# piotrprzybyszdev/Path-Tracing

Measured on AMD Instinct MI355X. Metric: Msamples/s (paths*spp/s) at 1920x1080, 8spp, depth 8, higher is better.
Workload: dtype f32; 1 GPU; chess_like (procedural stand-in for BASELINE configs[1] 'Khronos ABeautifulGame'), 1920x1080, 8 spp, depth 8; triangles=1999000, frames_in_flight=8, parallelism=pixel-tile shard x1, backend=wavefront, tile=32

## Files before the change

### path-tracing_amd/csrc/pt_bvh.hpp

```cpp
#pragma once

#include "pt_device.hpp"

namespace ptd
{

constexpr int kNodeWidth = 4;
struct BvhNode
{
    float4 a;
    int4 refs;
    uint4 q0;
    uint4 q1;
};
static_assert(sizeof(BvhNode) == 64, "BvhNode is 64 B");
constexpr int kEmptyRef = 0x7ffffffe;
constexpr int kRefDone = 0x7fffffff;
constexpr int kRefNone = 0x7ffffffd;

struct Tri
{
    float4 a;
    float4 b;
    float4 c;
};
static_assert(sizeof(Tri) == 48, "Tri is 48 B");
constexpr uint32_t kTriNonOpaque = 0x80000000u;
constexpr uint32_t kLeafNonOpaque = 0x40000000u, kLeafSlotMask = 0x3fffffffu;
constexpr uint32_t kMaxTriangles = 0x3fffffffu;

struct Hit
{
    float t, u, v;
    uint32_t pair, prim;
    uint32_t slot;
};


constexpr uint32_t kRefillMin = 16;
constexpr int kLdsStack = 16;
constexpr int kLdsStackMega = 64;
constexpr int kGlobalSpill = 80;
constexpr uint32_t kMaxPersistentThreads = 2048u * 256u;
constexpr uint32_t kMaxNodeVisits = 1u << 20;

struct AlphaTri
{
    float4 a;
    float4 b;
};
struct AlphaTex
{
// ... 288 lines not shown
#endif
            if (kMaskWalk)
            {
                PT_ENTER_UNORDERED(h, r0, r1, r2, r3, st, ref, kRefNone, push)
            }
            else
            {
                if (h > 3) st.push((uint32_t)r3);
                if (h > 2) st.push((uint32_t)r2);
                if (h > 1) st.push((uint32_t)r1);
                ref = h > 0 ? r0 : kRefNone;
            }
            if (STATS && stackDepth && (uint32_t)st.sp > *stackDepth)
                *stackDepth = (uint32_t)st.sp;
            if (ref == kRefNone)
            {
                if (st.sp == 0)
                    break;
                ref = (int)st.pop();
            }
        }
        else
        {
            if (STATS)
                (*triTests)++;
            const uint32_t leafSlot = ALPHA ? (uint32_t)~ref & kLeafSlotMask : (uint32_t)~ref;
            const Tri *tp = &sc.tris[leafSlot];
            const float4 ta = tp->a, tb = tp->b, tc = tp->c;
            float t, u, v;
            if (intersectTri(F3(ta.x, ta.y, ta.z), F3(ta.w, tb.x, tb.y), F3(tb.z, tb.w, tc.x), o, d, tmin, tmax, t, u, v) &&
                (!ALPHA || !(__float_as_uint(tc.w) & kTriNonOpaque) ||
                 anyHitKeeps<ANY_HIT>(sc, __float_as_uint(tc.y), __float_as_uint(tc.z), leafSlot, __float_as_uint(tc.w), t, u, v, decal)))
            {
                const uint32_t pair = __float_as_uint(tc.y), prim = __float_as_uint(tc.z);
                if (ANY_HIT)
                {
                    best.pair = pair;
                    best.prim = prim;
                    best.slot = leafSlot;
                    return true;
                }
                if (t < best.t || (t == best.t && (pair < best.pair || (pair == best.pair && prim < best.prim))))
                {
                    best.t = t;
                    best.u = u;
                    best.v = v;
                    best.pair = pair;
                    best.prim = prim;
                    best.slot = leafSlot;
                }
            }
            if (st.sp == 0)
                break;
            ref = (int)st.pop();
        }
    }
    if (ALPHA && decalOut)
        *decalOut = decal;
    return best.pair != 0xffffffffu;
}

constexpr uint32_t kTraceChunk = 128;
constexpr int kNodeStepsPerRound = 2;


#define PT_TMIN (IO::kFixedTmin >= 0.0f ? IO::kFixedTmin : tmin)
#define PT_TMAX (IO::kFixedTmax >= 0.0f ? IO::kFixedTmax : tmax)
template <bool ANY_HIT, bool ALPHA, typename IO>
PT_DEV void persistentTrace(const TraceScene &sc, IO &io, uint32_t count, uint32_t *__restrict__ chunkCounter, Stack &st)
{
    const uint32_t lane = threadIdx.x & 63u;
    const uint64_t below = (1ull << lane) - 1ull;
// ... 108 lines not shown
                }
                else
                {
                    if (kUnordered)
                    {
                        PT_ENTER_UNORDERED(h, r0, r1, r2, r3, st, ref, kRefNone, push)
                    }
                    else
                    {
                        if (h > 3) st.push((uint32_t)r3);
                        if (h > 2) st.push((uint32_t)r2);
                        if (h > 1) st.push((uint32_t)r1);
                        ref = h > 0 ? r0 : kRefNone;
                    }
                    if (ref == kRefNone)
                        ref = st.sp ? (int)st.pop() : kRefDone;
                }
            }
        }

        if (have && ref < 0)
        {
            const uint32_t leafBits = (uint32_t)~ref;
            const uint32_t leafSlot = ALPHA ? leafBits & kLeafSlotMask : leafBits;
            const Tri *tp = &sc.tris[leafSlot];
            const float4 ta = tp->a, tb = tp->b, tc = tp->c;
            float4 aa = make_float4(0.0f, 0.0f, 0.0f, 0.0f), ab = aa;
            const bool nonOpaque = ALPHA && (leafBits & kLeafNonOpaque) != 0u;
            if (nonOpaque)
            {
                aa = sc.alphaTris[leafSlot].a;
                ab = sc.alphaTris[leafSlot].b;
            }
            float t, u, v;
            if (__builtin_expect(st.allInLds(), 1))
                ref = st.sp ? (int)st.popLds() : kRefDone;
            else
                ref = st.sp ? (int)st.pop() : kRefDone;
            bool candidate = intersectTri(F3(ta.x, ta.y, ta.z), F3(ta.w, tb.x, tb.y), F3(tb.z, tb.w, tc.x), o, d, PT_TMIN, PT_TMAX, t, u, v);
            uint32_t pair = __float_as_uint(tc.y), prim = __float_as_uint(tc.z);
            if (ALPHA && candidate && nonOpaque)
            {
                const float alpha = hitAlpha(sc, aa, ab, __float_as_uint(tc.w), u, v);
                candidate = ANY_HIT ? !(alpha < 1.0f) : !(alpha < 0.5f);
                if (!ANY_HIT && !candidate && t <= best.t)
                    io.ignored(t, u, v, leafSlot, sc);
                if (candidate && (!ANY_HIT || IO::kNeedsPrim))
                {
                    const float4 again = sc.tris[fetchAgainAfter(leafSlot, alpha)].c;
                    pair = __float_as_uint(again.y);
                    prim = __float_as_uint(again.z);
                }
            }
            if (candidate)
            {
                if (ANY_HIT)
                {
                    best.pair = IO::kNeedsPrim ? pair : 0u;
                    best.slot = leafSlot;
                    ref = kRefDone;
                }
                else if (t < best.t || (t == best.t && (pair < best.pair || (pair == best.pair && prim < __float_as_uint(sc.tris[io.bestSlot(item)].c.z)))))
                {
// ... 22 lines not shown
```

### path-tracing_amd/csrc/pt_bvh_build.hpp

```cpp
#pragma once

#include "pt_bvh.hpp"

namespace ptd
{


PT_DEV uint32_t orderedFloat(float f)
{
    const uint32_t u = __float_as_uint(f);
    return (u & 0x80000000u) ? ~u : (u | 0x80000000u);
}
PT_DEV float unorderedFloat(uint32_t u)
{
    return __uint_as_float((u & 0x80000000u) ? (u & 0x7fffffffu) : ~u);
}

__global__ void k_tri_setup(uint32_t n, uint32_t pairCount, const uint32_t *__restrict__ pairFirst,
                            const DevPair *__restrict__ pairs, const PtxVertex *__restrict__ vertices,
                            const uint32_t *__restrict__ indices, Tri *__restrict__ triTmp, float4 *__restrict__ boxLo,
                            float4 *__restrict__ boxHi, uint32_t *__restrict__ sceneBounds, uint8_t *__restrict__ inert, int refit)
{
    const uint32_t g = blockIdx.x * blockDim.x + threadIdx.x;
    if (g >= n)
// ... 47 lines not shown
    boxHi[g] = make_float4(h[0], h[1], h[2], 0.0f);
    if (refit)
        return;
    for (int a = 0; a < 3; a++)
    {
        const float c = 0.5f * (l[a] + h[a]);
        const bool ok = !isInert && c == c && fabsf(c) < 3.0e38f;
        uint32_t mn = ok ? orderedFloat(c) : 0xffffffffu, mx = ok ? orderedFloat(c) : 0u;
        const bool fullWave = __ballot(1) == ~0ull;
        if (fullWave)
            for (int o = 32; o > 0; o >>= 1)
            {
                mn = min(mn, (uint32_t)__shfl_xor((int)mn, o));
                mx = max(mx, (uint32_t)__shfl_xor((int)mx, o));
            }
        if (!fullWave || (threadIdx.x & 63u) == 0u)
        {
            if (mn != 0xffffffffu)
                atomicMin(&sceneBounds[a], mn);
            if (mx != 0u)
                atomicMax(&sceneBounds[3 + a], mx);
        }
    }
}

constexpr uint32_t kMaxSplitsPerTri = 64;
constexpr double kSplitPriorityScale = 1048576.0;

struct SplitGrid
{
    float mn[3], cell[3];
};
PT_DEV SplitGrid splitGrid(const uint32_t *sceneBounds, int cubic)
{
    SplitGrid g;
    float widest = 0.0f;
    for (int a = 0; a < 3; a++)
        widest = fmaxf(widest, unorderedFloat(sceneBounds[3 + a]) - unorderedFloat(sceneBounds[a]));
    for (int a = 0; a < 3; a++)
    {
        g.mn[a] = unorderedFloat(sceneBounds[a]);
        const float ext = cubic ? widest : unorderedFloat(sceneBounds[3 + a]) - g.mn[a];
        g.cell[a] = ext > 0.0f ? ext / 2097152.0f : 0.0f;
    }
    return g;
}
// ... 1139 lines not shown
        d[8] = v->Tangent[0]; d[9] = v->Tangent[1]; d[10] = v->Tangent[2];
        d[11] = v->Bitangent[0]; d[12] = v->Bitangent[1]; d[13] = v->Bitangent[2];
        o[k] = loadVertex(v);
    }
    f[42] = f[43] = 0.0f;
    f3 wp[3], wn[3], gn;
    worldCorners(pr, o[0], o[1], o[2], wp, wn, gn);
    for (int k = 0; k < 3; k++)
    {
        f[44 + 3 * k] = wp[k].x; f[45 + 3 * k] = wp[k].y; f[46 + 3 * k] = wp[k].z;
        f[53 + 3 * k] = wn[k].x; f[54 + 3 * k] = wn[k].y; f[55 + 3 * k] = wn[k].z;
    }
    f[62] = gn.x; f[63] = gn.y; f[64] = gn.z;
    f[65] = f[66] = f[67] = 0.0f;
    for (int k = 0; k < 17; k++)
        out->v[k] = make_float4(f[4 * k], f[4 * k + 1], f[4 * k + 2], f[4 * k + 3]);
}

__global__ void k_emit(int n, const uint32_t *__restrict__ vals, const float4 *__restrict__ boxLo,
                       const float4 *__restrict__ boxHi, const int2 *__restrict__ children, const float4 *__restrict__ nodeLo,
                       const float4 *__restrict__ nodeHi, const Tri *__restrict__ triTmp, BvhNode *__restrict__ nodes,
                       Tri *__restrict__ tris, const DevPair *__restrict__ pairs, const PtxVertex *__restrict__ vertices,
                       const uint32_t *__restrict__ indices, ShadeTri *__restrict__ shadeTris, const uint8_t *__restrict__ decide,
                       const uint32_t *__restrict__ refTri)
{
    const int i = blockIdx.x * blockDim.x + threadIdx.x;
    if (i < n)
    {
        const Tri t = triTmp[refTri ? refTri[vals[i]] : vals[i]];
        tris[i] = t;
        writeShadeTri(t, pairs, vertices, indices, &shadeTris[i]);
    }
    if (i >= n - 1)
        return;
    ChildBox c[kNodeWidth];
    int count = 2;
    if (decide)
    {
        int ref[kNodeWidth] = { 0, 0, 0, 0 }, slots[kNodeWidth] = { 0, 0, 0, 0 }, sp = 0, out[kNodeWidth] = { 0, 0, 0, 0 };
        count = 0;
        {
            const int2 ch = children[i];
            const int k = 1 + (int)((decide[i] >> 1) & 3u);
            ref[0] = ch.y; slots[0] = 4 - k;
            ref[1] = ch.x; slots[1] = k;
            sp = 2;
        }
        while (sp > 0)
        {
            sp--;
            const int x = ref[sp], j = slots[sp];
            const uint32_t d = x >= 0 ? decide[x] : 0u;
            if (x < 0 || j == 1 || ((d >> (1 + j)) & 1u))
                out[count++] = x;
// ... 103 lines not shown
                    while (qh < 255 && decodeQ(o[a], qh, scale) < (double)c[k].hi[a])
                        qh++;
                    if (decodeQ(o[a], qh, scale) < (double)c[k].hi[a])
                        ok = false;
                }
                {
                    wl |= ql << (8 * k);
                    wh |= qh << (8 * k);
                }
            }
            if (ok || e >= 254)
            {
                ebits[a] = (uint32_t)e;
                qlo[a] = wl;
                qhi[a] = wh;
                break;
            }
            e++;
        }
    }
    BvhNode nd;
    nd.a = make_float4(o[0], o[1], o[2], __uint_as_float(ebits[0] | (ebits[1] << 8) | (ebits[2] << 16) | (orderAxis << 24)));
    for (int k = 0; k < count; k++)
        if (c[k].ref < 0 && (__float_as_uint(triTmp[refTri ? refTri[vals[~c[k].ref]] : vals[~c[k].ref]].c.w) & kTriNonOpaque))
            c[k].ref = ~(int)((uint32_t)~c[k].ref | kLeafNonOpaque);
    nd.refs = make_int4(c[0].ref, c[1].ref, count > 2 ? c[2].ref : kEmptyRef, count > 3 ? c[3].ref : kEmptyRef);
    nd.q0 = make_uint4(qlo[0], qhi[0], qlo[1], qhi[1]);
    nd.q1 = make_uint4(qlo[2], qhi[2], 0u, 0u);
    nodes[i] = nd;
}

__global__ void __launch_bounds__(256) k_relayout_level(uint32_t lo, uint32_t hi, const BvhNode *__restrict__ raw, uint32_t *__restrict__ oldOf,
                                                        uint32_t *__restrict__ nextFree, BvhNode *__restrict__ out)
{
    const uint32_t i = lo + blockIdx.x * blockDim.x + threadIdx.x, lane = threadIdx.x & 63u;
    BvhNode nd;
    nd.refs = make_int4(kEmptyRef, kEmptyRef, kEmptyRef, kEmptyRef);
    if (i < hi)
        nd = raw[oldOf[i]];
    int refs[kNodeWidth] = { nd.refs.x, nd.refs.y, nd.refs.z, nd.refs.w };
    uint32_t c = 0;
    for (int k = 0; k < kNodeWidth; k++)
        c += (refs[k] >= 0 && refs[k] != kEmptyRef) ? 1u : 0u;
    uint32_t incl = c;
    for (uint32_t d = 1; d < 64; d <<= 1)
    {
        const uint32_t up = __shfl_up(incl, d);
        if (lane >= d)
// ... 41 lines not shown
        pos[0] = 0u;
    for (int k = 0; k < kNodeWidth; k++)
        if (refs[k] >= 0 && refs[k] != kEmptyRef)
        {
            pos[refs[k]] = next;
            next += size[refs[k]];
        }
}
__global__ void k_place_nodes(uint32_t count, const BvhNode *__restrict__ nodes, const uint32_t *__restrict__ pos, BvhNode *__restrict__ out)
{
    const uint32_t i = blockIdx.x * blockDim.x + threadIdx.x;
    if (i >= count)
        return;
    BvhNode nd = nodes[i];
    int refs[kNodeWidth] = { nd.refs.x, nd.refs.y, nd.refs.z, nd.refs.w };
    for (int k = 0; k < kNodeWidth; k++)
        if (refs[k] >= 0 && refs[k] != kEmptyRef)
            refs[k] = (int)pos[refs[k]];
    nd.refs = make_int4(refs[0], refs[1], refs[2], refs[3]);
    out[pos[i]] = nd;
}

__global__ void k_single_leaf_root(const uint32_t *vals, const float4 *boxLo, const float4 *boxHi, const Tri *triTmp, BvhNode *nodes, Tri *tris,
                                   const DevPair *pairs, const PtxVertex *vertices, const uint32_t *indices, ShadeTri *shadeTris)
{
    const uint32_t g = vals[0];
    writeShadeTri(triTmp[g], pairs, vertices, indices, &shadeTris[0]);
    tris[0] = triTmp[g];
    BvhNode nd;
    const float lo[3] = { boxLo[g].x, boxLo[g].y, boxLo[g].z }, hi[3] = { boxHi[g].x, boxHi[g].y, boxHi[g].z };
    uint32_t eb[3];
    for (int a = 0; a < 3; a++)
    {
        int e = 1;
        while (e < 254 && decodeQ(lo[a], 255u, __uint_as_float((uint32_t)e << 23)) < (double)hi[a])
            e++;
        eb[a] = (uint32_t)e;
    }
    nd.a = make_float4(lo[0], lo[1], lo[2], __uint_as_float(eb[0] | (eb[1] << 8) | (eb[2] << 16)));
    nd.refs = make_int4((__float_as_uint(triTmp[g].c.w) & kTriNonOpaque) ? ~(int)kLeafNonOpaque : ~0, kEmptyRef, kEmptyRef, kEmptyRef);
    nd.q0 = make_uint4(0xffffff00u, 0x000000ffu, 0xffffff00u, 0x000000ffu);
    nd.q1 = make_uint4(0xffffff00u, 0x000000ffu, 0u, 0u);
    nodes[0] = nd;
}

__global__ void k_alpha_tris(uint32_t n, Tri *__restrict__ tris, const ShadeTri *__restrict__ shadeTris, SceneView sv,
                             const uint32_t *__restrict__ alphaTexOf, const AlphaTex *__restrict__ alphaTex, AlphaTri *__restrict__ out)
{
    const uint32_t i = blockIdx.x * blockDim.x + threadIdx.x;
    if (i >= n)
        return;
    AlphaTri r;
    r.a = make_float4(0.0f, 0.0f, 0.0f, 0.0f);
    r.b = make_float4(0.0f, 0.0f, 1.0f, __uint_as_float(kNoAlphaTex));
    const float4 tc = tris[i].c;
    if (__float_as_uint(tc.w) & kTriNonOpaque)
    {
        const ShadeTri *st = &shadeTris[i];
        const float4 q0 = st->v[0], q1 = st->v[1], q4 = st->v[4], q7 = st->v[7], q8 = st->v[8];
        r.a = make_float4(q0.w, q1.x, q4.y, q4.z);
        const DevPair *pr = &sv.pairs[__float_as_uint(tc.y)];
        const uint32_t materialType = pr->materialId & 0xffu, materialIndex = pr->materialId >> 8;
        uint32_t idx = 0;
// ... 42 lines not shown
```

### path-tracing_amd/csrc/pt_runtime.hpp

```cpp
#pragma once

#include <algorithm>
#include <atomic>
#include <cstdarg>
#include <cstdio>
#include <cstdlib>
#include <cstring>
#include <string>
#include <vector>

#include "pt_aux_kernels.hpp"
#include "pt_bvh_build.hpp"
#include "pt_post.hpp"


template <typename T> struct DevBuf
{
    T *p = nullptr;
    size_t n = 0;
    DevBuf() = default;
    DevBuf(const DevBuf &) = delete;
    DevBuf &operator=(const DevBuf &) = delete;
    ~DevBuf() { release(); }
    hipError_t alloc(size_t count)
// ... 35 lines not shown
};

struct EnvSwitches
{
    uint32_t cuPartition = 0;
    bool singleStream = false;
    bool verbose = false;
    bool karrasBuilder = false;
    bool plocFixed = false;
    uint32_t plocRadius = 0;
    float plocShape = 0.0f;
    int reinsertPasses = -1;
    float splitBudget = -1.0f;
    int layout = -1;
    int collapse = -1;
    int shadeSort = -1;
    long tailThreshold = -1;
    uint32_t framesPerWave = 8;
    uint32_t raysPerThread = 0;
    long residentCap = -1;
    uint32_t copyGroups = 0;
    bool snapshotMemcpy = false;
    bool fenceRefit = false;
    static EnvSwitches read()
    {
        EnvSwitches e;
        e.verbose = getenv("PTX_VERBOSE") != nullptr;
        if (const char *v = getenv("PTX_COPY_GROUPS"))
            e.copyGroups = (uint32_t)strtoul(v, nullptr, 10);
        e.snapshotMemcpy = getenv("PTX_SNAPSHOT_MEMCPY") != nullptr && std::strcmp(getenv("PTX_SNAPSHOT_MEMCPY"), "0") != 0;
        e.fenceRefit = getenv("PTX_FENCE_REFIT") != nullptr && std::strcmp(getenv("PTX_FENCE_REFIT"), "0") != 0;
        if (const char *v = getenv("PTX_BUILDER"))
            e.karrasBuilder = std::strcmp(v, "lbvh") == 0;
        if (const char *v = getenv("PTX_PLOC_SHAPE"))
        {
            e.plocFixed = true;
            e.plocShape = (float)atof(v);
        }
        if (const char *v = getenv("PTX_PLOC_RADIUS"))
        {
            e.plocFixed = true;
            e.plocRadius = std::max(1u, (uint32_t)strtoul(v, nullptr, 10));
        }
        if (const char *v = getenv("PTX_REINSERT"))
            e.reinsertPasses = atoi(v);
        if (const char *v = getenv("PTX_SPLIT_BUDGET"))
            e.splitBudget = (float)atof(v);
        if (const char *v = getenv("PTX_NODE_LAYOUT"))
            e.layout = atoi(v) ? 1 : 0;
        if (const char *v = getenv("PTX_COLLAPSE"))
// ... 43 lines not shown
    DevBuf<uint32_t> alphaTexOf;
    DevBuf<float4> alphaQuads;
    DevBuf<AlphaTri> alphaTris;
    uint32_t textureCount = 0;
    uint32_t skyKind = PTX_SKYBOX_CLEAR_COLOR;
    bool samplerNeeded = false;
    std::vector<DevPair> hostPairs;
    std::vector<uint32_t> pairInstance;
    std::vector<PtxTransform> pairMeshTransform;
    uint32_t instanceCount = 0, skinnedCount = 0, boneCount = 0;
    uint64_t staticVertexCount = 0;
    DevBuf<PtxAnimatedVertex> animatedVertices;
    DevBuf<uint32_t> skinSource;
    DevBuf<PtxTransform> bones;
    struct BuildState
    {
        DevBuf<Tri> triTmp;
        DevBuf<float4> boxLo, boxHi, nodeLo, nodeHi;
        DevBuf<uint32_t> sceneBounds, vals0, vals1, hist, histSums, flags;
        DevBuf<uint8_t> inert;
        DevBuf<float4> refLo, refHi;
        DevBuf<uint32_t> refTri;
        DevBuf<uint8_t> refInert;
        uint32_t refCount = 0;
        uint32_t treeTris = 0;
        DevBuf<uint64_t> keys0, keys1;
        DevBuf<int2> children;
        DevBuf<int> parentOfNode, parentOfLeaf;
        DevBuf<BvhNode> rawNodes;
        DevBuf<float4> collapseCost;
        DevBuf<uint8_t> collapseDecide;
        DevBuf<uint32_t> oldOf;
        DevBuf<uint32_t> lvDepth0, lvDepth1, lvVals0, lvVals1, lvStartDev;
        DevBuf<int> lvAnc0, lvAnc1;
        const uint32_t *levelOrder = nullptr;
        std::vector<uint32_t> levelStart;
        bool levelsValid = false;
        bool valid = false;
        void release()
        {
            triTmp.release(); boxLo.release(); boxHi.release(); nodeLo.release(); nodeHi.release(); sceneBounds.release();
            vals0.release(); vals1.release(); hist.release(); histSums.release(); flags.release(); inert.release(); keys0.release(); keys1.release();
            children.release(); parentOfNode.release(); parentOfLeaf.release(); rawNodes.release(); oldOf.release(); collapseCost.release(); collapseDecide.release();
            refLo.release(); refHi.release(); refTri.release(); refInert.release();
            lvDepth0.release(); lvDepth1.release(); lvVals0.release(); lvVals1.release(); lvStartDev.release(); lvAnc0.release(); lvAnc1.release();
            levelOrder = nullptr; levelStart.clear(); levelsValid = false;
            valid = false;
        }
    } build;
    bool anyNonOpaque = false;
    bool mixedMaterialTypes = false;
    bool mixedTextured = false;
    bool usePloc = true;
    TreeParams tree;
    bool reinsertBroken = false;
    uint32_t residentClosest[2] = { 0, 0 }, residentShadow[2] = { 0, 0 };
    DevBuf<float4> decal;
    DevBuf<float> decalT;
    size_t decalCapacity = 0;
    uint32_t pairCount = 0, triCount = 0, dxNormalTextures = 0;
    uint32_t treeTris = 0;
    bool sceneReady = false, accelReady = false;
    PtxRenderer *sceneOwner = nullptr;
    std::vector<PtxRenderer *> sceneSharers;

    DevBuf<BvhNode> nodes;
    DevBuf<Tri> tris;
// ... 518 lines not shown
            pr.vertexOffset = geo.VertexOffset;
            pr.indexOffset = geo.IndexOffset;
            if (geo.IsAnimated)
            {
                if (s->vertexCount + skinSource.size() + geo.VertexLength > 0xffffffffull || s->indexCount + s->animatedIndexCount > 0xffffffffull)
                    return fail(r, PTX_ERROR_INVALID_ARGUMENT, "animated meshes exceed the 32-bit vertex / index space");
                pr.vertexOffset = static_cast<uint32_t>(s->vertexCount + skinSource.size());
                pr.indexOffset = static_cast<uint32_t>(s->indexCount + geo.IndexOffset);
                for (uint32_t v = 0; v < geo.VertexLength; v++)
                    skinSource.push_back(geo.VertexOffset + v);
            }
            r->pairInstance.push_back(i);
            r->pairMeshTransform.push_back(s->transforms[rec.TransformIndex]);
            pr.materialId = rec.MaterialId;
            pr.flags = (geo.IsOpaque ? 0u : kPairNonOpaque) | (materialSamplesSceneTexture(s, rec.MaterialId) ? kPairTextured : 0u);
            if (pr.flags & kPairNonOpaque)
                anyNonOpaque = true;
            pairs.push_back(pr);
            pairFirst.push_back(static_cast<uint32_t>(tri));
            tri += geo.IndexLength / 3;
        }
    }
    if (tri > kMaxTriangles)
        return fail(r, PTX_ERROR_INVALID_ARGUMENT, "scene has %llu triangles; limit is 2^30-1", (unsigned long long)tri);
    pairFirst.push_back(static_cast<uint32_t>(tri));
    {
        uint32_t typesSeen = 0;
        for (const DevPair &pr : pairs)
            typesSeen |= 1u << ((pr.materialId & 0xffu) <= PTX_MATERIAL_TYPE_PHONG ? (pr.materialId & 0xffu) : 3u);
        r->mixedMaterialTypes = (typesSeen & (typesSeen - 1u)) != 0u;
        bool textured = false, plain = false;
        for (const DevPair &pr : pairs)
            ((pr.flags & kPairTextured) ? textured : plain) = true;
        r->mixedTextured = textured && plain;
    }
    r->pairCount = static_cast<uint32_t>(pairs.size());
    r->triCount = static_cast<uint32_t>(tri);
    r->dxNormalTextures = s->dxNormalTextures;

    int rc;
    r->hostPairs = pairs;
    r->instanceCount = s->instanceCount;
    r->staticVertexCount = s->vertexCount;
    r->skinnedCount = static_cast<uint32_t>(skinSource.size());
    r->boneCount = 0;
    r->build.release();
    std::vector<PtxVertex> verts;
// ... 454 lines not shown
            if (sb > 1)
            {
                k_scan32_sums<<<sb, 256, 0, r->stream>>>(nTri + 1, count.p, sums.p);
                k_scan_exclusive<<<1, 1024, 0, r->stream>>>(sb, sums.p);
                k_scan32_apply<<<sb, 256, 0, r->stream>>>(nTri + 1, count.p, sums.p);
            }
            else
                k_scan_exclusive<<<1, 1024, 0, r->stream>>>(nTri + 1, count.p);
            uint32_t refs = 0;
            BUILD_TRY(hipMemcpyAsync(&refs, count.p + nTri, sizeof(refs), hipMemcpyDeviceToHost, r->stream));
            BUILD_TRY(hipStreamSynchronize(r->stream));
            if (refs > nTri && refs <= kMaxTriangles)
            {
                BUILD_TRY(B.refLo.alloc(refs)); BUILD_TRY(B.refHi.alloc(refs)); BUILD_TRY(B.refTri.alloc(refs)); BUILD_TRY(B.refInert.alloc(refs));
                k_split_write<<<(nTri + 255) / 256, 256, 0, r->stream>>>(nTri, B.triTmp.p, B.boxLo.p, B.boxHi.p, B.inert.p, B.sceneBounds.p,
                                                                        r->tree.mortonCubic ? 1 : 0, count.p, refs, B.refLo.p, B.refHi.p, B.refTri.p, B.refInert.p);
                BUILD_TRY(hipStreamSynchronize(r->stream));
                n = refs;
                refLo = B.refLo.p; refHi = B.refHi.p; refInert = B.refInert.p; refTri = B.refTri.p;
            }
        }
    }
    if (!refit)
        B.refCount = n;

    const uint32_t numTiles = (n + kSortTile - 1) / kSortTile;
    const uint32_t histCount = 256 * numTiles, histBlocks = (histCount + kScan32Block - 1) / kScan32Block;
    if (!refit)
    {
        BUILD_TRY(r->nodes.alloc(n));
        BUILD_TRY(r->tris.alloc(n));
        BUILD_TRY(r->shadeTris.alloc(n));
        BUILD_TRY(B.nodeLo.alloc(n)); BUILD_TRY(B.nodeHi.alloc(n)); BUILD_TRY(B.vals0.alloc(n)); BUILD_TRY(B.vals1.alloc(n));
        BUILD_TRY(B.hist.alloc(histCount)); BUILD_TRY(B.histSums.alloc(histBlocks)); BUILD_TRY(B.flags.alloc(n));
        BUILD_TRY(B.keys0.alloc(n)); BUILD_TRY(B.keys1.alloc(n));
        BUILD_TRY(B.children.alloc(n)); BUILD_TRY(B.parentOfNode.alloc(n)); BUILD_TRY(B.parentOfLeaf.alloc(n));
        BUILD_TRY(B.rawNodes.alloc(n)); BUILD_TRY(B.oldOf.alloc((size_t)n + 1)); BUILD_TRY(B.collapseCost.alloc(n)); BUILD_TRY(B.collapseDecide.alloc(n));
    }

    DevBuf<int> cl0, cl1;
    DevBuf<float4> lo0, hi0, lo1, hi1;
    DevBuf<uint32_t> nn;
    DevBuf<unsigned long long> flags, sums, total;
    if (!refit && r->usePloc && n > 1)
    {
        BUILD_TRY(cl0.alloc(n)); BUILD_TRY(cl1.alloc(n)); BUILD_TRY(lo0.alloc(n)); BUILD_TRY(hi0.alloc(n)); BUILD_TRY(lo1.alloc(n));
        BUILD_TRY(hi1.alloc(n)); BUILD_TRY(nn.alloc(n)); BUILD_TRY(flags.alloc(n)); BUILD_TRY(sums.alloc((n + kScanBlock - 1) / kScanBlock));
        BUILD_TRY(total.alloc(1));
    }
    BUILD_TRY(hipMemsetAsync(B.flags.p, 0, (size_t)n * 4, r->stream));

    const uint32_t blocks = (n + 255) / 256;
    uint64_t *kin = B.keys0.p, *kout = B.keys1.p;
    uint32_t *vin = B.vals0.p, *vout = B.vals1.p;
    uint32_t nv = B.treeTris;
    if (!refit)
    {
        k_morton<<<blocks, 256, 0, r->stream>>>(n, refLo, refHi, B.sceneBounds.p, refInert, B.keys0.p, B.vals0.p, r->tree.mortonCubic ? 1 : 0);
        for (uint32_t shift = 0; shift < 64; shift += 8)
        {
            k_sort_hist<<<numTiles, 64, 0, r->stream>>>(n, kin, shift, numTiles, B.hist.p);
            if (histBlocks > 1)
            {
                k_scan32_sums<<<histBlocks, 256, 0, r->stream>>>(histCount, B.hist.p, B.histSums.p);
                k_scan_exclusive<<<1, 1024, 0, r->stream>>>(histBlocks, B.histSums.p);
                k_scan32_apply<<<histBlocks, 256, 0, r->stream>>>(histCount, B.hist.p, B.histSums.p);
            }
            else
                k_scan_exclusive<<<1, 1024, 0, r->stream>>>(histCount, B.hist.p);
            k_sort_scatter<<<numTiles, 64, 0, r->stream>>>(n, kin, vin, kout, vout, shift, numTiles, B.hist.p);
            std::swap(kin, kout);
            std::swap(vin, vout);
        }
        k_count_valid<<<1, 1, 0, r->stream>>>(n, kin, &B.sceneBounds.p[6]);
        BUILD_TRY(hipMemcpyAsync(&nv, &B.sceneBounds.p[6], sizeof(nv), hipMemcpyDeviceToHost, r->stream));
        BUILD_TRY(hipStreamSynchronize(r->stream));
        B.treeTris = nv;
    }
    r->treeTris = nv;
    r->stats.bvhNodes = nv > 1 ? nv - 1 : (nv ? 1 : 0);
    r->stats.treeReferences = nv;
    r->stats.treeTriangles = nTri - (n - nv);
    const uint32_t vblocks = (nv + 255) / 256;
    if (nv == 1)
        k_single_leaf_root<<<1, 1, 0, r->stream>>>(vin, refLo, refHi, B.triTmp.p, r->nodes.p, r->tris.p, r->pairs.p, r->vertices.p,
                                                   r->indices.p, r->shadeTris.p);
    else if (nv > 1)
    {
        bool boxesDone = false;
        if (!refit && r->usePloc)
        {
            k_ploc_init<<<vblocks, 256, 0, r->stream>>>(nv, vin, refLo, refHi, cl0.p, lo0.p, hi0.p);
            int *cIn = cl0.p, *cOut = cl1.p;
            float4 *lIn = lo0.p, *hIn = hi0.p, *lOut = lo1.p, *hOut = hi1.p;
            uint32_t count = nv;
            int nextId = (int)nv - 2;
            uint32_t iterations = 0;
            while (count > 1)
            {
                const uint32_t cb = (count + 255) / 256, sb = (count + kScanBlock - 1) / kScanBlock;
                k_ploc_nearest<<<cb, 256, 0, r->stream>>>(count, r->tree.plocRadius, r->tree.plocShape, lIn, hIn, nn.p);
                k_ploc_flags<<<cb, 256, 0, r->stream>>>(count, nn.p, flags.p);
                k_scan64_sums<<<sb, 256, 0, r->stream>>>(count, flags.p, sums.p);
                k_scan64_top<<<1, 1024, 0, r->stream>>>(sb, sums.p, total.p);
                k_scan64_apply<<<sb, 256, 0, r->stream>>>(count, flags.p, sums.p);
                k_ploc_merge<<<cb, 256, 0, r->stream>>>(count, cIn, lIn, hIn, nn.p, flags.p, nextId, cOut, lOut, hOut, B.children.p, B.parentOfNode.p,
                                                        B.parentOfLeaf.p, B.nodeLo.p, B.nodeHi.p);
                unsigned long long t = 0;
                BUILD_TRY(hipMemcpyAsync(&t, total.p, sizeof(t), hipMemcpyDeviceToHost, r->stream));
// ... 85 lines not shown
            }
            BUILD_TRY(hipStreamSynchronize(r->stream));
        }
        if (r->tree.collapse)
        {
            if (!refit && !B.levelsValid && !fenceKernels)
                BUILD_TRY(treeLevels(r, nv, &haveLevels));
            if (B.levelsValid && !fenceKernels)
                for (size_t d = B.levelStart.size() - 1; d-- > 0;)
                {
                    const uint32_t first = B.levelStart[d], count = B.levelStart[d + 1] - first;
                    k_collapse_cost_level<<<(count + 255) / 256, 256, 0, r->stream>>>(first, count, B.levelOrder, vin, refLo, refHi, B.children.p, B.nodeLo.p,
                                                                                     B.nodeHi.p, B.collapseCost.p, B.collapseDecide.p);
                }
            else
            {
                BUILD_TRY(hipMemsetAsync(B.flags.p, 0, (size_t)nv * 4, r->stream));
                k_collapse_cost<<<vblocks, 256, 0, r->stream>>>((int)nv, vin, refLo, refHi, B.children.p, B.parentOfNode.p, B.parentOfLeaf.p, B.nodeLo.p, B.nodeHi.p,
                                                           B.flags.p, B.collapseCost.p, B.collapseDecide.p);
            }
        }
        k_emit<<<vblocks, 256, 0, r->stream>>>((int)nv, vin, refLo, refHi, B.children.p, B.nodeLo.p, B.nodeHi.p, B.triTmp.p,
                                              B.rawNodes.p, r->tris.p, r->pairs.p, r->vertices.p, r->indices.p, r->shadeTris.p,
                                              r->tree.collapse ? B.collapseDecide.p : nullptr, refTri);
        uint32_t *nextFree = B.oldOf.p + n;
        const uint32_t first[1] = { 0u }, one = 1u;
        BUILD_TRY(hipMemcpyAsync(B.oldOf.p, first, sizeof(first), hipMemcpyHostToDevice, r->stream));
        BUILD_TRY(hipMemcpyAsync(nextFree, &one, sizeof(one), hipMemcpyHostToDevice, r->stream));
        uint32_t lo = 0, hi = 1, levels = 0;
        std::vector<uint32_t> levelStart;
        while (lo < hi)
        {
            levelStart.push_back(lo);
            k_relayout_level<<<(hi - lo + 255) / 256, 256, 0, r->stream>>>(lo, hi, B.rawNodes.p, B.oldOf.p, nextFree, r->nodes.p);
            uint32_t end = 0;
            BUILD_TRY(hipMemcpyAsync(&end, nextFree, sizeof(end), hipMemcpyDeviceToHost, r->stream));
            BUILD_TRY(hipStreamSynchronize(r->stream));
            if (end < hi || end > nv - 1)
            {
                B.release();
                return fail(r, PTX_ERROR_DEVICE, "ptx_build_accel: relayout placed %u nodes of at most %u", end, nv - 1);
            }
            lo = hi;
            hi = end;
            levels++;
        }
        r->stats.bvhNodes = hi;
        if (r->tree.layout == 1 && hi > 1)
        {
            levelStart.push_back(hi);
            uint32_t *size = B.flags.p, *pos = B.vals1.p == vin ? B.vals0.p : B.vals1.p;
            for (uint32_t l = levels; l-- > 0;)
                k_subtree_size<<<(levelStart[l + 1] - levelStart[l] + 255) / 256, 256, 0, r->stream>>>(levelStart[l], levelStart[l + 1], r->nodes.p, size);
            for (uint32_t l = 0; l < levels; l++)
                k_subtree_pos<<<(levelStart[l + 1] - levelStart[l] + 255) / 256, 256, 0, r->stream>>>(levelStart[l], levelStart[l + 1], r->nodes.p, size, pos);
            k_place_nodes<<<(hi + 255) / 256, 256, 0, r->stream>>>(hi, r->nodes.p, pos, B.rawNodes.p);
            r->nodes.swap(B.rawNodes);
        }
        if (r->env.verbose)
            std::fprintf(stderr, "[ptx] relayout: %u of %u emitted nodes are live, %u levels\n", hi, nv - 1, levels);
    }
    if (r->anyNonOpaque && nv)
    {
        BUILD_TRY(r->alphaTris.alloc(n));
        k_alpha_tris<<<vblocks, 256, 0, r->stream>>>(nv, r->tris.p, r->shadeTris.p, makeSceneView(r), r->alphaTexOf.p, r->alphaTex.p, r->alphaTris.p);
    }
    uint32_t revived = 0;
    if (refit)
        BUILD_TRY(hipMemcpyAsync(&revived, &B.sceneBounds.p[7], sizeof(revived), hipMemcpyDeviceToHost, r->stream));
    BUILD_TRY(hipEventRecord(r->evB, r->stream));
    BUILD_TRY(hipStreamSynchronize(r->stream));
    BUILD_TRY(hipGetLastError());
    if (revived)
        return buildAccel(r, false, keepState);
    float ms = 0.0f;
    (void)hipEventElapsedTime(&ms, r->evA, r->evB);
    r->stats.lastBuildMs = ms;
    if (keepState)
        B.valid = true;
    else
        B.release();
#undef BUILD_TRY
    r->accelReady = true;
    return PTX_OK;
}

static TraceScene makeTraceScene(const PtxRenderer *r);

// ... 963 lines not shown
```

Measured before the change: 2389 Msamples/s.

## Pair adjacent edge-sharing triangles into two-triangle BVH leaves

During the BVH build, adjacent opaque triangles from the same mesh that share an edge, and whose union box is no larger than the sum of their boxes, are merged into one leaf reference. The leaf carries a pair bit and traversal tests both triangles stored in consecutive slots. This shrinks the tree, cutting node count and node visits per ray. The cost is a second triangle fetch and test at paired leaves, extra build passes (pointer jumping and scans), and one fewer bit of triangle index range.

```diff
diff --git a/path-tracing_amd/csrc/pt_bvh.hpp b/path-tracing_amd/csrc/pt_bvh.hpp
--- a/path-tracing_amd/csrc/pt_bvh.hpp
+++ b/path-tracing_amd/csrc/pt_bvh.hpp
@@ -26,8 +26,8 @@
 };
 static_assert(sizeof(Tri) == 48, "Tri is 48 B");
 constexpr uint32_t kTriNonOpaque = 0x80000000u;
-constexpr uint32_t kLeafNonOpaque = 0x40000000u, kLeafSlotMask = 0x3fffffffu;
-constexpr uint32_t kMaxTriangles = 0x3fffffffu;
+constexpr uint32_t kLeafNonOpaque = 0x40000000u, kLeafPair = 0x20000000u, kLeafSlotMask = 0x1fffffffu;
+constexpr uint32_t kMaxTriangles = 0x1fffffffu;
 
 struct Hit
 {
@@ -362,32 +362,38 @@
         }
         else
         {
+            const uint32_t leafBits = (uint32_t)~ref, firstSlot = leafBits & kLeafSlotMask;
+            const uint32_t tests = (leafBits & kLeafPair) ? 2u : 1u;
             if (STATS)
-                (*triTests)++;
-            const uint32_t leafSlot = ALPHA ? (uint32_t)~ref & kLeafSlotMask : (uint32_t)~ref;
-            const Tri *tp = &sc.tris[leafSlot];
-            const float4 ta = tp->a, tb = tp->b, tc = tp->c;
-            float t, u, v;
-            if (intersectTri(F3(ta.x, ta.y, ta.z), F3(ta.w, tb.x, tb.y), F3(tb.z, tb.w, tc.x), o, d, tmin, tmax, t, u, v) &&
-                (!ALPHA || !(__float_as_uint(tc.w) & kTriNonOpaque) ||
-                 anyHitKeeps<ANY_HIT>(sc, __float_as_uint(tc.y), __float_as_uint(tc.z), leafSlot, __float_as_uint(tc.w), t, u, v, decal)))
-            {
-                const uint32_t pair = __float_as_uint(tc.y), prim = __float_as_uint(tc.z);
-                if (ANY_HIT)
-                {
-                    best.pair = pair;
-                    best.prim = prim;
-                    best.slot = leafSlot;
-                    return true;
-                }
-                if (t < best.t || (t == best.t && (pair < best.pair || (pair == best.pair && prim < best.prim))))
-                {
-                    best.t = t;
-                    best.u = u;
-                    best.v = v;
-                    best.pair = pair;
-                    best.prim = prim;
-                    best.slot = leafSlot;
+                (*triTests) += tests;
+#pragma nounroll
+            for (uint32_t k = 0; k < tests; k++)
+            {
+                const uint32_t leafSlot = firstSlot + k;
+                const Tri *tp = &sc.tris[leafSlot];
+                const float4 ta = tp->a, tb = tp->b, tc = tp->c;
+                float t, u, v;
+                if (intersectTri(F3(ta.x, ta.y, ta.z), F3(ta.w, tb.x, tb.y), F3(tb.z, tb.w, tc.x), o, d, tmin, tmax, t, u, v) &&
+                    (!ALPHA || !(__float_as_uint(tc.w) & kTriNonOpaque) ||
+                     anyHitKeeps<ANY_HIT>(sc, __float_as_uint(tc.y), __float_as_uint(tc.z), leafSlot, __float_as_uint(tc.w), t, u, v, decal)))
+                {
+                    const uint32_t pair = __float_as_uint(tc.y), prim = __float_as_uint(tc.z);
+                    if (ANY_HIT)
+                    {
+                        best.pair = pair;
+                        best.prim = prim;
+                        best.slot = leafSlot;
+                        return true;
+                    }
+                    if (t < best.t || (t == best.t && (pair < best.pair || (pair == best.pair && prim < best.prim))))
+                    {
+                        best.t = t;
+                        best.u = u;
+                        best.v = v;
+                        best.pair = pair;
+                        best.prim = prim;
+                        best.slot = leafSlot;
+                    }
                 }
             }
             if (st.sp == 0)
@@ -542,9 +548,10 @@
         if (have && ref < 0)
         {
             const uint32_t leafBits = (uint32_t)~ref;
-            const uint32_t leafSlot = ALPHA ? leafBits & kLeafSlotMask : leafBits;
+            uint32_t leafSlot = leafBits & kLeafSlotMask;
             const Tri *tp = &sc.tris[leafSlot];
             const float4 ta = tp->a, tb = tp->b, tc = tp->c;
+            const bool pairLeaf = (leafBits & kLeafPair) != 0u;
             float4 aa = make_float4(0.0f, 0.0f, 0.0f, 0.0f), ab = aa;
             const bool nonOpaque = ALPHA && (leafBits & kLeafNonOpaque) != 0u;
             if (nonOpaque)
@@ -559,6 +566,17 @@
                 ref = st.sp ? (int)st.pop() : kRefDone;
             bool candidate = intersectTri(F3(ta.x, ta.y, ta.z), F3(ta.w, tb.x, tb.y), F3(tb.z, tb.w, tc.x), o, d, PT_TMIN, PT_TMAX, t, u, v);
             uint32_t pair = __float_as_uint(tc.y), prim = __float_as_uint(tc.z);
+            if (pairLeaf && !(ANY_HIT && candidate))
+            {
+                const float4 sa = tp[1].a, sb = tp[1].b;
+                const float sc2 = tp[1].c.x;
+                if (intersectTri(F3(sa.x, sa.y, sa.z), F3(sa.w, sb.x, sb.y), F3(sb.z, sb.w, sc2), o, d, PT_TMIN, candidate ? t : PT_TMAX, t, u, v))
+                {
+                    candidate = true;
+                    prim++;
+                    leafSlot++;
+                }
+            }
             if (ALPHA && candidate && nonOpaque)
             {
                 const float alpha = hitAlpha(sc, aa, ab, __float_as_uint(tc.w), u, v);
diff --git a/path-tracing_amd/csrc/pt_bvh_build.hpp b/path-tracing_amd/csrc/pt_bvh_build.hpp
--- a/path-tracing_amd/csrc/pt_bvh_build.hpp
+++ b/path-tracing_amd/csrc/pt_bvh_build.hpp
@@ -93,6 +93,97 @@
                 atomicMax(&sceneBounds[3 + a], mx);
         }
     }
+}
+
+constexpr float kPairAreaFactor = 1.0f;
+
+PT_DEV float boxArea4(float4 lo, float4 hi)
+{
+    const float dx = hi.x - lo.x, dy = hi.y - lo.y, dz = hi.z - lo.z;
+    return dx * dy + dy * dz + dz * dx;
+}
+
+__global__ void k_pair_links(uint32_t n, const Tri *__restrict__ triTmp, const DevPair *__restrict__ pairs, const uint32_t *__restrict__ indices,
+                             const float4 *__restrict__ boxLo, const float4 *__restrict__ boxHi, const uint8_t *__restrict__ inert,
+                             uint8_t *__restrict__ link)
+{
+    const uint32_t g = blockIdx.x * blockDim.x + threadIdx.x;
+    if (g >= n)
+        return;
+    bool ok = false;
+    if (g + 1 < n && !inert[g] && !inert[g + 1])
+    {
+        const float4 c0 = triTmp[g].c, c1 = triTmp[g + 1].c;
+        const uint32_t p = __float_as_uint(c0.y), prim = __float_as_uint(c0.z);
+        ok = p == __float_as_uint(c1.y) && !((__float_as_uint(c0.w) | __float_as_uint(c1.w)) & kTriNonOpaque);
+        if (ok)
+        {
+            const uint32_t *ia = &indices[pairs[p].indexOffset + prim * 3];
+            uint32_t shared = 0;
+            for (int a = 0; a < 3; a++)
+                for (int b = 0; b < 3; b++)
+                    shared += ia[a] == ia[3 + b] ? 1u : 0u;
+            const float4 l0 = boxLo[g], h0 = boxHi[g], l1 = boxLo[g + 1], h1 = boxHi[g + 1];
+            const float4 lu = make_float4(fminf(l0.x, l1.x), fminf(l0.y, l1.y), fminf(l0.z, l1.z), 0.0f);
+            const float4 hu = make_float4(fmaxf(h0.x, h1.x), fmaxf(h0.y, h1.y), fmaxf(h0.z, h1.z), 0.0f);
+            ok = shared >= 2 && boxArea4(lu, hu) <= kPairAreaFactor * (boxArea4(l0, h0) + boxArea4(l1, h1));
+        }
+    }
+    link[g] = ok ? 1 : 0;
+}
+
+__global__ void k_pair_jump(uint32_t n, const uint8_t *__restrict__ link, const uint32_t *__restrict__ in, uint32_t *__restrict__ out)
+{
+    const uint32_t g = blockIdx.x * blockDim.x + threadIdx.x;
+    if (g >= n)
+        return;
+    out[g] = in ? in[in[g]] : (g > 0 && link[g - 1] ? g - 1 : g);
+}
+
+PT_DEV bool pairsWithNext(uint32_t g, const uint8_t *link, const uint32_t *start) { return link[g] && ((g - start[g]) & 1u) == 0u; }
+__global__ void k_pair_heads(uint32_t n, const uint8_t *__restrict__ link, const uint32_t *__restrict__ start, uint32_t *__restrict__ head)
+{
+    const uint32_t g = blockIdx.x * blockDim.x + threadIdx.x;
+    if (g >= n)
+        return;
+    head[g] = (g > 0 && pairsWithNext(g - 1, link, start)) ? 0u : 1u;
+}
+
+__global__ void k_pair_write(uint32_t n, const uint8_t *__restrict__ link, const uint32_t *__restrict__ start, const uint32_t *__restrict__ refIndex,
+                             const uint8_t *__restrict__ inert, uint32_t *__restrict__ refTri, uint8_t *__restrict__ refPair, uint8_t *__restrict__ refInert)
+{
+    const uint32_t g = blockIdx.x * blockDim.x + threadIdx.x;
+    if (g >= n || refIndex[g + 1] == refIndex[g])
+        return;
+    const uint32_t r = refIndex[g];
+    refTri[r] = g;
+    refPair[r] = pairsWithNext(g, link, start) ? 1 : 0;
+    refInert[r] = inert[g];
+}
+
+__global__ void k_ref_boxes(uint32_t n, const uint32_t *__restrict__ refTri, const uint8_t *__restrict__ refPair, const float4 *__restrict__ boxLo,
+                            const float4 *__restrict__ boxHi, float4 *__restrict__ refLo, float4 *__restrict__ refHi)
+{
+    const uint32_t r = blockIdx.x * blockDim.x + threadIdx.x;
+    if (r >= n)
+        return;
+    const uint32_t g = refTri[r];
+    float4 lo = boxLo[g], hi = boxHi[g];
+    if (refPair[r])
+    {
+        const float4 l1 = boxLo[g + 1], h1 = boxHi[g + 1];
+        lo = make_float4(fminf(lo.x, l1.x), fminf(lo.y, l1.y), fminf(lo.z, l1.z), 0.0f);
+        hi = make_float4(fmaxf(hi.x, h1.x), fmaxf(hi.y, h1.y), fmaxf(hi.z, h1.z), 0.0f);
+    }
+    refLo[r] = lo;
+    refHi[r] = hi;
+}
+
+__global__ void k_slot_sizes(uint32_t nv, const uint32_t *__restrict__ vals, const uint8_t *__restrict__ refPair, uint32_t *__restrict__ sizes)
+{
+    const uint32_t i = blockIdx.x * blockDim.x + threadIdx.x;
+    if (i <= nv)
+        sizes[i] = i < nv ? 1u + (uint32_t)refPair[vals[i]] : 0u;
 }
 
 constexpr uint32_t kMaxSplitsPerTri = 64;
@@ -1278,14 +1369,21 @@
                        const float4 *__restrict__ nodeHi, const Tri *__restrict__ triTmp, BvhNode *__restrict__ nodes,
                        Tri *__restrict__ tris, const DevPair *__restrict__ pairs, const PtxVertex *__restrict__ vertices,
                        const uint32_t *__restrict__ indices, ShadeTri *__restrict__ shadeTris, const uint8_t *__restrict__ decide,
-                       const uint32_t *__restrict__ refTri)
+                       const uint32_t *__restrict__ refTri, const uint32_t *__restrict__ slotOf, const uint8_t *__restrict__ refPair)
 {
     const int i = blockIdx.x * blockDim.x + threadIdx.x;
     if (i < n)
     {
-        const Tri t = triTmp[refTri ? refTri[vals[i]] : vals[i]];
-        tris[i] = t;
-        writeShadeTri(t, pairs, vertices, indices, &shadeTris[i]);
+        const uint32_t g = refTri ? refTri[vals[i]] : vals[i], s = slotOf ? slotOf[i] : (uint32_t)i;
+        const Tri t = triTmp[g];
+        tris[s] = t;
+        writeShadeTri(t, pairs, vertices, indices, &shadeTris[s]);
+        if (refPair && refPair[vals[i]])
+        {
+            const Tri t2 = triTmp[g + 1];
+            tris[s + 1] = t2;
+            writeShadeTri(t2, pairs, vertices, indices, &shadeTris[s + 1]);
+        }
     }
     if (i >= n - 1)
         return;
@@ -1435,8 +1533,16 @@
     BvhNode nd;
     nd.a = make_float4(o[0], o[1], o[2], __uint_as_float(ebits[0] | (ebits[1] << 8) | (ebits[2] << 16) | (orderAxis << 24)));
     for (int k = 0; k < count; k++)
-        if (c[k].ref < 0 && (__float_as_uint(triTmp[refTri ? refTri[vals[~c[k].ref]] : vals[~c[k].ref]].c.w) & kTriNonOpaque))
-            c[k].ref = ~(int)((uint32_t)~c[k].ref | kLeafNonOpaque);
+        if (c[k].ref < 0)
+        {
+            const uint32_t pos = (uint32_t)~c[k].ref, r = vals[pos];
+            uint32_t bits = slotOf ? slotOf[pos] : pos;
+            if (__float_as_uint(triTmp[refTri ? refTri[r] : r].c.w) & kTriNonOpaque)
+                bits |= kLeafNonOpaque;
+            if (refPair && refPair[r])
+                bits |= kLeafPair;
+            c[k].ref = ~(int)bits;
+        }
     nd.refs = make_int4(c[0].ref, c[1].ref, count > 2 ? c[2].ref : kEmptyRef, count > 3 ? c[3].ref : kEmptyRef);
     nd.q0 = make_uint4(qlo[0], qhi[0], qlo[1], qhi[1]);
     nd.q1 = make_uint4(qlo[2], qhi[2], 0u, 0u);
@@ -1524,13 +1630,21 @@
 }
 
 __global__ void k_single_leaf_root(const uint32_t *vals, const float4 *boxLo, const float4 *boxHi, const Tri *triTmp, BvhNode *nodes, Tri *tris,
-                                   const DevPair *pairs, const PtxVertex *vertices, const uint32_t *indices, ShadeTri *shadeTris)
-{
-    const uint32_t g = vals[0];
+                                   const DevPair *pairs, const PtxVertex *vertices, const uint32_t *indices, ShadeTri *shadeTris,
+                                   const uint32_t *refTri, const uint8_t *refPair)
+{
+    const uint32_t r = vals[0];
+    const uint32_t g = refTri ? refTri[r] : r;
+    const bool pair = refPair && refPair[r];
     writeShadeTri(triTmp[g], pairs, vertices, indices, &shadeTris[0]);
     tris[0] = triTmp[g];
+    if (pair)
+    {
+        writeShadeTri(triTmp[g + 1], pairs, vertices, indices, &shadeTris[1]);
+        tris[1] = triTmp[g + 1];
+    }
     BvhNode nd;
-    const float lo[3] = { boxLo[g].x, boxLo[g].y, boxLo[g].z }, hi[3] = { boxHi[g].x, boxHi[g].y, boxHi[g].z };
+    const float lo[3] = { boxLo[r].x, boxLo[r].y, boxLo[r].z }, hi[3] = { boxHi[r].x, boxHi[r].y, boxHi[r].z };
     uint32_t eb[3];
     for (int a = 0; a < 3; a++)
     {
@@ -1540,7 +1654,8 @@
         eb[a] = (uint32_t)e;
     }
     nd.a = make_float4(lo[0], lo[1], lo[2], __uint_as_float(eb[0] | (eb[1] << 8) | (eb[2] << 16)));
-    nd.refs = make_int4((__float_as_uint(triTmp[g].c.w) & kTriNonOpaque) ? ~(int)kLeafNonOpaque : ~0, kEmptyRef, kEmptyRef, kEmptyRef);
+    const uint32_t bits = ((__float_as_uint(triTmp[g].c.w) & kTriNonOpaque) ? kLeafNonOpaque : 0u) | (pair ? kLeafPair : 0u);
+    nd.refs = make_int4(~(int)bits, kEmptyRef, kEmptyRef, kEmptyRef);
     nd.q0 = make_uint4(0xffffff00u, 0x000000ffu, 0xffffff00u, 0x000000ffu);
     nd.q1 = make_uint4(0xffffff00u, 0x000000ffu, 0u, 0u);
     nodes[0] = nd;
diff --git a/path-tracing_amd/csrc/pt_runtime.hpp b/path-tracing_amd/csrc/pt_runtime.hpp
--- a/path-tracing_amd/csrc/pt_runtime.hpp
+++ b/path-tracing_amd/csrc/pt_runtime.hpp
@@ -81,10 +81,13 @@
     uint32_t copyGroups = 0;
     bool snapshotMemcpy = false;
     bool fenceRefit = false;
+    bool pairLeaves = true;
     static EnvSwitches read()
     {
         EnvSwitches e;
         e.verbose = getenv("PTX_VERBOSE") != nullptr;
+        if (const char *v = getenv("PTX_PAIR_LEAVES"))
+            e.pairLeaves = std::strcmp(v, "0") != 0;
         if (const char *v = getenv("PTX_COPY_GROUPS"))
             e.copyGroups = (uint32_t)strtoul(v, nullptr, 10);
         e.snapshotMemcpy = getenv("PTX_SNAPSHOT_MEMCPY") != nullptr && std::strcmp(getenv("PTX_SNAPSHOT_MEMCPY"), "0") != 0;
@@ -174,6 +177,9 @@
         DevBuf<float4> refLo, refHi;
         DevBuf<uint32_t> refTri;
         DevBuf<uint8_t> refInert;
+        DevBuf<uint8_t> refPair;
+        DevBuf<uint32_t> slotOf;
+        bool pairRefs = false;
         uint32_t refCount = 0;
         uint32_t treeTris = 0;
         DevBuf<uint64_t> keys0, keys1;
@@ -194,7 +200,7 @@
             triTmp.release(); boxLo.release(); boxHi.release(); nodeLo.release(); nodeHi.release(); sceneBounds.release();
             vals0.release(); vals1.release(); hist.release(); histSums.release(); flags.release(); inert.release(); keys0.release(); keys1.release();
             children.release(); parentOfNode.release(); parentOfLeaf.release(); rawNodes.release(); oldOf.release(); collapseCost.release(); collapseDecide.release();
-            refLo.release(); refHi.release(); refTri.release(); refInert.release();
+            refLo.release(); refHi.release(); refTri.release(); refInert.release(); refPair.release(); slotOf.release(); pairRefs = false;
             lvDepth0.release(); lvDepth1.release(); lvVals0.release(); lvVals1.release(); lvStartDev.release(); lvAnc0.release(); lvAnc1.release();
             levelOrder = nullptr; levelStart.clear(); levelsValid = false;
             valid = false;
@@ -759,7 +765,7 @@
         }
     }
     if (tri > kMaxTriangles)
-        return fail(r, PTX_ERROR_INVALID_ARGUMENT, "scene has %llu triangles; limit is 2^30-1", (unsigned long long)tri);
+        return fail(r, PTX_ERROR_INVALID_ARGUMENT, "scene has %llu triangles; limit is 2^29-1", (unsigned long long)tri);
     pairFirst.push_back(static_cast<uint32_t>(tri));
     {
         uint32_t typesSeen = 0;
@@ -1260,6 +1266,53 @@
         }
     }
     if (!refit)
+    {
+        B.pairRefs = false;
+        if (r->env.pairLeaves && r->tree.splitBudget <= 0.0f && nTri > 1)
+        {
+            DevBuf<uint8_t> link;
+            DevBuf<uint32_t> s0, s1, head, sums;
+            const uint32_t sb = (nTri + 1 + kScan32Block - 1) / kScan32Block, tb = (nTri + 255) / 256;
+            BUILD_TRY(link.alloc(nTri)); BUILD_TRY(s0.alloc(nTri)); BUILD_TRY(s1.alloc(nTri)); BUILD_TRY(head.alloc((size_t)nTri + 1)); BUILD_TRY(sums.alloc(sb));
+            k_pair_links<<<tb, 256, 0, r->stream>>>(nTri, B.triTmp.p, r->pairs.p, r->indices.p, B.boxLo.p, B.boxHi.p, B.inert.p, link.p);
+            k_pair_jump<<<tb, 256, 0, r->stream>>>(nTri, link.p, nullptr, s0.p);
+            for (uint32_t span = 1; span < nTri; span *= 2)
+            {
+                k_pair_jump<<<tb, 256, 0, r->stream>>>(nTri, link.p, s0.p, s1.p);
+                s0.swap(s1);
+            }
+            BUILD_TRY(hipMemsetAsync(head.p + nTri, 0, sizeof(uint32_t), r->stream));
+            k_pair_heads<<<tb, 256, 0, r->stream>>>(nTri, link.p, s0.p, head.p);
+            if (sb > 1)
+            {
+                k_scan32_sums<<<sb, 256, 0, r->stream>>>(nTri + 1, head.p, sums.p);
+                k_scan_exclusive<<<1, 1024, 0, r->stream>>>(sb, sums.p);
+                k_scan32_apply<<<sb, 256, 0, r->stream>>>(nTri + 1, head.p, sums.p);
+            }
+            else
+                k_scan_exclusive<<<1, 1024, 0, r->stream>>>(nTri + 1, head.p);
+            uint32_t refs = 0;
+            BUILD_TRY(hipMemcpyAsync(&refs, head.p + nTri, sizeof(refs), hipMemcpyDeviceToHost, r->stream));
+            BUILD_TRY(hipStreamSynchronize(r->stream));
+            if (refs < nTri)
+            {
+                BUILD_TRY(B.refLo.alloc(refs)); BUILD_TRY(B.refHi.alloc(refs)); BUILD_TRY(B.refTri.alloc(refs)); BUILD_TRY(B.refInert.alloc(refs));
+                BUILD_TRY(B.refPair.alloc(refs)); BUILD_TRY(B.slotOf.alloc((size_t)refs + 1));
+                k_pair_write<<<tb, 256, 0, r->stream>>>(nTri, link.p, s0.p, head.p, B.inert.p, B.refTri.p, B.refPair.p, B.refInert.p);
+                BUILD_TRY(hipStreamSynchronize(r->stream));
+                n = refs;
+                B.pairRefs = true;
+            }
+        }
+    }
+    if (B.pairRefs)
+    {
+        k_ref_boxes<<<(n + 255) / 256, 256, 0, r->stream>>>(n, B.refTri.p, B.refPair.p, B.boxLo.p, B.boxHi.p, B.refLo.p, B.refHi.p);
+        refLo = B.refLo.p; refHi = B.refHi.p; refInert = B.refInert.p; refTri = B.refTri.p;
+    }
+    const uint8_t *refPair = B.pairRefs ? B.refPair.p : nullptr;
+    const uint32_t slotCap = std::max(n, nTri);
+    if (!refit)
         B.refCount = n;
 
     const uint32_t numTiles = (n + kSortTile - 1) / kSortTile;
@@ -1267,8 +1320,8 @@
     if (!refit)
     {
         BUILD_TRY(r->nodes.alloc(n));
-        BUILD_TRY(r->tris.alloc(n));
-        BUILD_TRY(r->shadeTris.alloc(n));
+        BUILD_TRY(r->tris.alloc(slotCap));
+        BUILD_TRY(r->shadeTris.alloc(slotCap));
         BUILD_TRY(B.nodeLo.alloc(n)); BUILD_TRY(B.nodeHi.alloc(n)); BUILD_TRY(B.vals0.alloc(n)); BUILD_TRY(B.vals1.alloc(n));
         BUILD_TRY(B.hist.alloc(histCount)); BUILD_TRY(B.histSums.alloc(histBlocks)); BUILD_TRY(B.flags.alloc(n));
         BUILD_TRY(B.keys0.alloc(n)); BUILD_TRY(B.keys1.alloc(n));
@@ -1314,15 +1367,34 @@
         BUILD_TRY(hipMemcpyAsync(&nv, &B.sceneBounds.p[6], sizeof(nv), hipMemcpyDeviceToHost, r->stream));
         BUILD_TRY(hipStreamSynchronize(r->stream));
         B.treeTris = nv;
-    }
-    r->treeTris = nv;
+        if (B.pairRefs)
+        {
+            const uint32_t sb = (nv + 1 + kScan32Block - 1) / kScan32Block;
+            DevBuf<uint32_t> sums;
+            BUILD_TRY(sums.alloc(sb));
+            k_slot_sizes<<<(nv + 1 + 255) / 256, 256, 0, r->stream>>>(nv, vin, B.refPair.p, B.slotOf.p);
+            if (sb > 1)
+            {
+                k_scan32_sums<<<sb, 256, 0, r->stream>>>(nv + 1, B.slotOf.p, sums.p);
+                k_scan_exclusive<<<1, 1024, 0, r->stream>>>(sb, sums.p);
+                k_scan32_apply<<<sb, 256, 0, r->stream>>>(nv + 1, B.slotOf.p, sums.p);
+            }
+            else
+                k_scan_exclusive<<<1, 1024, 0, r->stream>>>(nv + 1, B.slotOf.p);
+            BUILD_TRY(hipStreamSynchronize(r->stream));
+        }
+    }
+    const uint32_t pairLeaves = B.pairRefs ? nTri - n : 0u, slots = nv + pairLeaves;
+    r->treeTris = slots;
     r->stats.bvhNodes = nv > 1 ? nv - 1 : (nv ? 1 : 0);
-    r->stats.treeReferences = nv;
+    r->stats.treeReferences = slots;
     r->stats.treeTriangles = nTri - (n - nv);
+    if (r->env.verbose && !refit && B.pairRefs)
+        std::fprintf(stderr, "[ptx] pair leaves: %u (%u of %u tree triangles paired)\n", pairLeaves, 2 * pairLeaves, slots);
     const uint32_t vblocks = (nv + 255) / 256;
     if (nv == 1)
         k_single_leaf_root<<<1, 1, 0, r->stream>>>(vin, refLo, refHi, B.triTmp.p, r->nodes.p, r->tris.p, r->pairs.p, r->vertices.p,
-                                                   r->indices.p, r->shadeTris.p);
+                                                   r->indices.p, r->shadeTris.p, refTri, refPair);
     else if (nv > 1)
     {
         bool boxesDone = false;
@@ -1454,7 +1526,7 @@
         }
         k_emit<<<vblocks, 256, 0, r->stream>>>((int)nv, vin, refLo, refHi, B.children.p, B.nodeLo.p, B.nodeHi.p, B.triTmp.p,
                                               B.rawNodes.p, r->tris.p, r->pairs.p, r->vertices.p, r->indices.p, r->shadeTris.p,
-                                              r->tree.collapse ? B.collapseDecide.p : nullptr, refTri);
+                                              r->tree.collapse ? B.collapseDecide.p : nullptr, refTri, B.pairRefs ? B.slotOf.p : nullptr, refPair);
         uint32_t *nextFree = B.oldOf.p + n;
         const uint32_t first[1] = { 0u }, one = 1u;
         BUILD_TRY(hipMemcpyAsync(B.oldOf.p, first, sizeof(first), hipMemcpyHostToDevice, r->stream));
@@ -1494,8 +1566,8 @@
     }
     if (r->anyNonOpaque && nv)
     {
-        BUILD_TRY(r->alphaTris.alloc(n));
-        k_alpha_tris<<<vblocks, 256, 0, r->stream>>>(nv, r->tris.p, r->shadeTris.p, makeSceneView(r), r->alphaTexOf.p, r->alphaTex.p, r->alphaTris.p);
+        BUILD_TRY(r->alphaTris.alloc(slotCap));
+        k_alpha_tris<<<(slots + 255) / 256, 256, 0, r->stream>>>(slots, r->tris.p, r->shadeTris.p, makeSceneView(r), r->alphaTexOf.p, r->alphaTex.p, r->alphaTris.p);
     }
     uint32_t revived = 0;
     if (refit)
```

Measured after the change: 2474 Msamples/s (median of 6 runs). 1.04x the previous value.
